# YongonY/NBLDPC

Measured on AMD Instinct MI355X. Metric: decoded codewords/sec @ 50 iters, GF(256) N=512 rate-1/2, higher is better.
Workload: dtype f64

## Files before the change

### nbldpc_amd/csrc/nbl_cn_ems256.hip

```cpp
#include <hip/hip_runtime.h>
#ifndef NBL_EMS_PRUNE
#define NBL_EMS_PRUNE 1
#endif
#ifndef NBL_EMS_ND
#define NBL_EMS_ND 1
#endif
#include <type_traits>
#include "nbl_device.h"
#include "nbl_kernels.h"

#ifndef NBL_WHATIF
#define NBL_WHATIF 0
#endif

namespace {

constexpr int Q = 256;

struct ListEnt { double v; int t8; int tt; };

#define WSYNC() __builtin_amdgcn_fence(__ATOMIC_ACQ_REL, "wavefront")

template <int CTRL, int ROW_MASK = 0xF>
__device__ __forceinline__ double dpp_mov_f64(double x)
{
	int lo = __builtin_amdgcn_update_dpp(__double2loint(x), __double2loint(x), CTRL, ROW_MASK, 0xF, false);
	int hi = __builtin_amdgcn_update_dpp(__double2hiint(x), __double2hiint(x), CTRL, ROW_MASK, 0xF, false);
	return __hiloint2double(hi, lo);
}

__device__ __forceinline__ double wave_max_f64(double x)
{
	x = dmax(x, dpp_mov_f64<0xB1>(x));
	x = dmax(x, dpp_mov_f64<0x4E>(x));
	x = dmax(x, dpp_mov_f64<0x141>(x));
	x = dmax(x, dpp_mov_f64<0x140>(x));
	x = dmax(x, dpp_mov_f64<0x142, 0xA>(x));
	x = dmax(x, dpp_mov_f64<0x143, 0xC>(x));
	return read_lane_f64(x, 63);
}

__device__ __forceinline__ int wave_scan_add(int x)
{
	x += __builtin_amdgcn_update_dpp(0, x, 0x111, 0xF, 0xF, false);
	x += __builtin_amdgcn_update_dpp(0, x, 0x112, 0xF, 0xF, false);
	x += __builtin_amdgcn_update_dpp(0, x, 0x114, 0xF, 0xF, false);
	x += __builtin_amdgcn_update_dpp(0, x, 0x118, 0xF, 0xF, false);
	x += __builtin_amdgcn_update_dpp(0, x, 0x142, 0xA, 0xF, false);
	x += __builtin_amdgcn_update_dpp(0, x, 0x143, 0xC, 0xF, false);
	return x;
}

__device__ __forceinline__ int wave_max_i32(int x)
{
	constexpr int ID = (int)0x80000000;
	auto mx = [](int a, int b) { return a > b ? a : b; };
	x = mx(x, __builtin_amdgcn_update_dpp(ID, x, 0xB1, 0xF, 0xF, false));
	x = mx(x, __builtin_amdgcn_update_dpp(ID, x, 0x4E, 0xF, 0xF, false));
	x = mx(x, __builtin_amdgcn_update_dpp(ID, x, 0x141, 0xF, 0xF, false));
	x = mx(x, __builtin_amdgcn_update_dpp(ID, x, 0x140, 0xF, 0xF, false));
	x = mx(x, __builtin_amdgcn_update_dpp(ID, x, 0x142, 0xA, 0xF, false));
	x = mx(x, __builtin_amdgcn_update_dpp(ID, x, 0x143, 0xC, 0xF, false));
	return __builtin_amdgcn_readlane(x, 63);
}
__device__ __forceinline__ int wave_min_i32(int x)
{
	constexpr int ID = 0x7fffffff;
	auto mn = [](int a, int b) { return a < b ? a : b; };
	x = mn(x, __builtin_amdgcn_update_dpp(ID, x, 0xB1, 0xF, 0xF, false));
	x = mn(x, __builtin_amdgcn_update_dpp(ID, x, 0x4E, 0xF, 0xF, false));
	x = mn(x, __builtin_amdgcn_update_dpp(ID, x, 0x141, 0xF, 0xF, false));
	x = mn(x, __builtin_amdgcn_update_dpp(ID, x, 0x140, 0xF, 0xF, false));
	x = mn(x, __builtin_amdgcn_update_dpp(ID, x, 0x142, 0xA, 0xF, false));
	x = mn(x, __builtin_amdgcn_update_dpp(ID, x, 0x143, 0xC, 0xF, false));
	return __builtin_amdgcn_readlane(x, 63);
}

__device__ __forceinline__ int key32(double x)
{
	const int b = __float_as_int((float)x);
	return b ^ ((b >> 31) & 0x7fffffff);
}
__device__ __forceinline__ float unkey32(int k) { return __int_as_float(k ^ ((k >> 31) & 0x7fffffff)); }

__device__ __forceinline__ double wave_max_exact(double loc, int key, int kmax)
{
	const uint64_t c = __ballot(key == kmax);
	if (__builtin_popcountll(c) == 1) return read_lane_f64(loc, __builtin_ctzll(c));
	return wave_max_f64(loc);
}

__device__ __forceinline__ int sym_of(int lane, int i) { return 2 * lane + (i & 1) + 128 * (i >> 1); }

__device__ __forceinline__ int highest_sym(const uint64_t (&m)[4])
{
	int best = -1;
#pragma unroll
	for (int i = 0; i < 4; i++) {
		if (m[i]) {
			int l = 63 - __builtin_clzll(m[i]);
			int a = 2 * l + (i & 1) + 128 * (i >> 1);
			best = a > best ? a : best;
		}
	}
	return best;
}
__device__ __forceinline__ int lowest_sym(const uint64_t (&m)[4])
{
	int best = Q;
#pragma unroll
	for (int i = 0; i < 4; i++) {
		if (m[i]) {
			int l = __builtin_ctzll(m[i]);
			int a = 2 * l + (i & 1) + 128 * (i >> 1);
			best = a < best ? a : best;
		}
	}
	return best;
}

struct GfMulL {
	int b0, b7, lane_part;
	__device__ __forceinline__ void init(int h, int poly, int lane)
	{
		int x = h;
		b0 = x;
		lane_part = 0;
#pragma unroll
		for (int i = 1; i < 8; i++) {
			x <<= 1;
			if (x & Q) x ^= poly;
			if (i < 7) lane_part ^= (-((lane >> (i - 1)) & 1)) & x;
			else b7 = x;
		}
	}
	__device__ __forceinline__ int at_slot(int i) const { return lane_part ^ ((i & 1) ? b0 : 0) ^ ((i & 2) ? b7 : 0); }
};

struct SelState {
	uint64_t cand[4];
	uint64_t gt[4], eq[4];
	int done;
};

__device__ __forceinline__ void select_step(const double (&v)[4], int nm, SelState &s)
{
	if (s.done) return;
	const uint64_t any = s.cand[0] | s.cand[1] | s.cand[2] | s.cand[3];
	if (!any) { s.done = 1; return; }
	double offer = __builtin_amdgcn_inverse_ballot_w64(s.cand[0]) ? v[0] : __builtin_amdgcn_inverse_ballot_w64(s.cand[1]) ? v[1]
	             : __builtin_amdgcn_inverse_ballot_w64(s.cand[2]) ? v[2] : v[3];
	const double pv = read_lane_f64(offer, __builtin_ctzll(any));
	uint64_t gt[4], ge[4];
	int cgt = 0, cge = 0;
#pragma unroll
	for (int i = 0; i < 4; i++) {
		gt[i] = __ballot(v[i] > pv);
		ge[i] = __ballot(v[i] >= pv);
		cgt += __popcll(gt[i]);
		cge += __popcll(ge[i]);
	}
	if (cgt >= nm) {
#pragma unroll
		for (int i = 0; i < 4; i++) s.cand[i] &= gt[i];
	} else if (cge >= nm) {
#pragma unroll
		for (int i = 0; i < 4; i++) { s.gt[i] = gt[i]; s.eq[i] = ge[i] & ~gt[i]; }
		s.done = 1;
	} else {
#pragma unroll
		for (int i = 0; i < 4; i++) s.cand[i] &= ~ge[i];
	}
}

__device__ __forceinline__ void finish_ties(uint64_t (&member)[4], const uint64_t (&eqin)[4], int need, int hinv, int poly, int lane)
{
	GfMulL mh;
	mh.init(hinv, poly, lane);
	uint64_t eq[4] = {eqin[0], eqin[1], eqin[2], eqin[3]};
	for (; need > 0; need--) {
		int best = -1;
#pragma unroll
		for (int i = 0; i < 4; i++) {
			const int a = __builtin_amdgcn_inverse_ballot_w64(eq[i]) ? mh.at_slot(i) : -1;
			best = a > best ? a : best;
		}
		const int amax = wave_max_i32(best);
#pragma unroll
		for (int i = 0; i < 4; i++) {
			const uint64_t hit = __ballot(__builtin_amdgcn_inverse_ballot_w64(eq[i]) && mh.at_slot(i) == amax);
			member[i] |= hit;
			eq[i] &= ~hit;
		}
	}
}

__device__ __forceinline__ void finish_members(SelState &s, int nm, uint64_t (&member)[4], int hinv, int poly, int lane)
{
	int cgt = 0, ceq = 0;
#pragma unroll
	for (int i = 0; i < 4; i++) { cgt += __popcll(s.gt[i]); ceq += __popcll(s.eq[i]); }
	const int need = nm - cgt;
#pragma unroll
	for (int i = 0; i < 4; i++) member[i] = s.gt[i];
	if (need == ceq) {
#pragma unroll
		for (int i = 0; i < 4; i++) member[i] |= s.eq[i];
	} else {
		finish_ties(member, s.eq, need, hinv, poly, lane);
	}
}

}

template <int NMT, bool FUSED, int NC>
__global__ __launch_bounds__(64) void cn_ems_q256_dc4_kernel(NblGraphDev g, NblWork w, NblRun r)
{
	constexpr int NM = NMT < 0 ? -NMT : NMT;
	constexpr bool VARNM = NMT < 0;
	const int nmr = VARNM ? r.nm : NM;
	constexpr int LOGNM = (NM == 8) ? 3 : (NM == 16) ? 4 : (NM == 32) ? 5 : 6;
#if NBL_WHATIF == 5
	__shared__ __attribute__((aligned(16))) char smem[13 * 1024];
#elif NBL_WHATIF == 6
	__shared__ __attribute__((aligned(16))) char smem[19 * 1024];
#else
	__shared__ __attribute__((aligned(16))) char smem[3 * Q * 8 + 4 * NM * 8 + 4 * NM * 8];
#endif
	const int lane = lane_id();
	const NblXcdSlot xs = nbl_xcd_slot(g.M);
	const int m = xs.unit, b = nbl_codeword(w, r, xs.slot);
	if (b < 0) return;
	if (!r.fixed_iters && w.done[b]) return;
#if NBL_EMS_PRUNE
	const bool tryf = NC >= 2 && r.fixed_iters && w.done[b];
#else
	const bool tryf = false;
#endif
	const int c0 = g.coff[m];

	double *const B0 = (double *)smem, *const B1 = B0 + Q, *const B2 = B1 + Q;
	double *const lstv = B2 + Q;
	int2 *const lstt = (int2 *)(lstv + 4 * NM);
	auto list_at = [&](int j, int k) {
		ListEnt e;
		e.v = lstv[j * NM + k];
		const int2 o = lstt[j * NM + k];
		e.t8 = o.x;
		e.tt = o.y;
		return e;
	};

#ifdef NBL_EMS_STAMPS
	unsigned long long st_t0 = 0, st_acc[15] = {0, 0, 0, 0, 0, 0, 0, 0, 0, 0, 0, 0, 0, 0, 0};
	const bool st_on = (w.stamps != nullptr) && ((blockIdx.x & 63) == 0);
#define STAMP(i) do { if (st_on) { unsigned long long t1_ = clock64(); st_acc[i] += t1_ - st_t0; st_t0 = t1_; } } while (0)
#define STAMP_COUNT(i) do { if (st_on) st_acc[i]++; } while (0)
	const unsigned long long st_begin = st_on ? clock64() : 0;
	unsigned long long st_mid = 0;
	int st_cls = 6;
	st_t0 = st_begin;
#elif defined(NBL_EMS_MARKS)
#define STAMP(i) asm volatile("; NBLMARK " #i)
#define STAMP_COUNT(i) do { } while (0)
#else
#define STAMP(i) do { } while (0)
#define STAMP_COUNT(i) do { } while (0)
#endif

	const double *V = w.v2c + (size_t)b * g.E * Q;
	double *C = w.c2v + ((size_t)b * g.E + c0) * Q;

	uint2 toff[4];
#define TOFF(j, i) ((int)((((i) & 2) ? toff[j].y : toff[j].x) >> (16 * ((i) & 1))) & 0xffff)
#pragma unroll
	for (int j = 0; j < 4; j++) toff[j] = ((const uint2 *)g.ems_toff)[(size_t)(c0 + j) * 64 + lane];

	double v[4][4];
	if (!FUSED) {
#pragma unroll
		for (int j = 0; j < 4; j++) {
			const double2 *src = (const double2 *)(V + (size_t)g.c_epos[c0 + j] * Q);
			double2 d0 = src[lane], d1 = src[64 + lane];
			v[j][0] = (lane == 0) ? 0.0 : d0.x;
			v[j][1] = d0.y;
			v[j][2] = d1.x;
			v[j][3] = d1.y;
		}
	} else {
		const double *Cp = w.c2v_prev + (w.c2v_prev_shared ? (size_t)0 : (size_t)b * g.E * Q);
		double2 l0[4], l1[4], a0[4], a1[4], b0[4], b1[4];
		int nvar[4], eidx[4];
		bool ownA[4];
		const int *row = g.dv2_row + (size_t)m * 16;
#pragma unroll
		for (int j = 0; j < 4; j++) {
			const int n = row[j], cpA = row[4 + j], cpB = row[8 + j], e = row[12 + j] & 0x7fffffff;
#if NBL_WHATIF == 11
			const double2 *pl = (const double2 *)(w.Lch + ((size_t)(b & 7) * g.N + n) * Q);
#else
			const double2 *pl = (const double2 *)(w.Lch + ((size_t)b * g.N + n) * Q);
#endif
			const double2 *pa = (const double2 *)(Cp + (size_t)cpA * Q);
			const double2 *pb = (const double2 *)(Cp + (size_t)cpB * Q);
#if NBL_WHATIF == 4
			l0[j].x = (double)(long long)(pl + lane) * -1e-9; l0[j].y = l0[j].x * 1.5; l1[j].x = l0[j].x * 0.7; l1[j].y = l0[j].x * 0.3;
			a0[j].x = (double)(long long)(pa + lane) * -1e-9; a0[j].y = a0[j].x * 1.25; a1[j].x = a0[j].x * 0.6; a1[j].y = a0[j].x * 0.2;
			b0[j].x = (double)(long long)(pb + lane) * -1e-9; b0[j].y = b0[j].x * 1.125; b1[j].x = b0[j].x * 0.9; b1[j].y = b0[j].x * 0.4;
#else
			l0[j] = pl[lane]; l1[j] = pl[64 + lane];
			a0[j] = pa[lane]; a1[j] = pa[64 + lane];
			b0[j] = pb[lane]; b1[j] = pb[64 + lane];
#endif
			nvar[j] = n; eidx[j] = e;
			ownA[j] = row[12 + j] < 0;
		}
#pragma unroll
		for (int j = 0; j < 4; j++) {
			const int n = nvar[j], e = eidx[j];
			double post[4] = {(l0[j].x + a0[j].x) + b0[j].x, (l0[j].y + a0[j].y) + b0[j].y, (l1[j].x + a1[j].x) + b1[j].x,
			                  (l1[j].y + a1[j].y) + b1[j].y};
			if (ownA[j]) {
				v[j][0] = post[0] - a0[j].x; v[j][1] = post[1] - a0[j].y; v[j][2] = post[2] - a1[j].x; v[j][3] = post[3] - a1[j].y;
			} else {
				asm volatile("");
				v[j][0] = post[0] - b0[j].x; v[j][1] = post[1] - b0[j].y; v[j][2] = post[2] - b1[j].x; v[j][3] = post[3] - b1[j].y;
			}
			if (lane == 0) v[j][0] = 0.0;
			if (ownA[j]) {
				if (lane == 0) post[0] = 0.0;
				const double locp = dmax(dmax(post[0], post[1]), dmax(post[2], post[3]));
				const int kp = key32(locp);
				const double pm = wave_max_exact(locp, kp, wave_max_i32(kp));
				uint64_t hit[4];
#pragma unroll
				for (int i = 0; i < 4; i++) hit[i] = __ballot(post[i] == pm);
				const int arg = lowest_sym(hit);
				if (lane == 0) w.dec[(size_t)b * g.N + n] = (pm > 0.0) ? arg : 0;
				if (w.post) {
					double2 *pp = (double2 *)(w.post + ((size_t)b * g.N + n) * Q);
					double2 p01, p23;
					p01.x = post[0]; p01.y = post[1]; p23.x = post[2]; p23.y = post[3];
					pp[lane] = p01;
					pp[64 + lane] = p23;
				}
			}
			if (w.store_v2c) {
				double2 *pv = (double2 *)(w.v2c + ((size_t)b * g.E + e) * Q);
				double2 v01, v23;
				v01.x = v[j][0]; v01.y = v[j][1]; v23.x = v[j][2]; v23.y = v[j][3];
				pv[lane] = v01;
				pv[64 + lane] = v23;
			}
		}
	}
	STAMP(0);

	double mtop[4], lmin[4];
	double sec[4] = {0, 0, 0, 0};
	int ztop[4];
#pragma unroll
	for (int j = 0; j < 4; j++) {
		const double loc = dmax(dmax(v[j][0], v[j][1]), dmax(v[j][2], v[j][3]));
		const int k = key32(loc);
		mtop[j] = wave_max_exact(loc, k, wave_max_i32(k));
		constexpr int KEY_3E38 = 0x7f61b1e6;
		const int kmin = wave_min_i32(k);
		const double lf = (double)unkey32(kmin < KEY_3E38 ? kmin : KEY_3E38);
		lmin[j] = ((lf - (mtop[j] - lf) * 0x1p-20) - __builtin_fabs(lf) * 0x1p-22) - 0x1p-120;
		uint64_t eqm[4];
#pragma unroll
		for (int i = 0; i < 4; i++) eqm[i] = __ballot(v[j][i] == mtop[j]);
		const int topa = highest_sym(eqm);
		const int tl = (topa & 127) >> 1;
		const unsigned twl = (unsigned)__builtin_amdgcn_readlane((int)toff[j].x, tl), twh = (unsigned)__builtin_amdgcn_readlane((int)toff[j].y, tl);
		const unsigned tw = (topa & 128) ? twh : twl;
		ztop[j] = (int)((tw >> (16 * (topa & 1))) & 0xffffu) >> 3;
#if NBL_EMS_PRUNE
		if (tryf) {
			const int ts = (topa & 1) + 2 * (topa >> 7);
			const double mate = (ts == 0) ? v[j][1] : (ts == 1) ? v[j][0] : (ts == 2) ? v[j][3] : v[j][2];
			const double far = (ts & 2) ? dmax(v[j][0], v[j][1]) : dmax(v[j][2], v[j][3]);
			const double loc2 = (lane == tl) ? dmax(mate, far) : loc;
			const double sf = (double)unkey32(wave_max_i32(key32(loc2)));
			sec[j] = uniform_f64((sf + __builtin_fabs(sf) * 0x1p-22) + 0x1p-120);
		}
#endif
	}
	STAMP(1);

	double S[4][4];
#pragma unroll
	for (int x = 0; x < 4; x++)
#pragma unroll
		for (int i = 0; i < 4; i++) S[x][i] = -NBL_DBL_MAX;
	const int ztot = ztop[0] ^ ztop[1] ^ ztop[2] ^ ztop[3];
	const int lane16 = lane << 4;
#pragma unroll
	for (int j = 0; j < 4; j++) {
		char *const Uj = (char *)(j == 1 ? B1 : j == 2 ? B2 : B0);
		WSYNC();
#pragma unroll
		for (int i = 0; i < 4; i++) *(double *)(Uj + TOFF(j, i)) = v[j][i];
		WSYNC();
#pragma unroll
		for (int x = 0; x < 4; x++) {
			if (x == j) continue;
			const int shift = ztot ^ ztop[x] ^ ztop[j];
			const int ad = lane16 ^ ((shift & 0xFE) << 3);
			const double2 ra = *(const double2 *)(Uj + ad), rb = *(const double2 *)(Uj + (ad ^ 1024));
			auto upd = [&](double u0, double u1, double u2, double u3) {
				const double uu[4] = {u0, u1, u2, u3};
#pragma unroll
				for (int i = 0; i < 4; i++) {
					double acc = 0.0;
#pragma unroll
					for (int o = 0; o < 4; o++) {
						if (o == x) continue;
						acc = acc + ((o == j) ? uu[i] : mtop[o]);
					}
					S[x][i] = dmax(S[x][i], acc);
				}
			};
			if (shift & 1) upd(ra.y, ra.x, rb.y, rb.x);
			else upd(ra.x, ra.y, rb.x, rb.y);
		}
		if (NC >= 2) {
			const double2 d0 = *(const double2 *)(Uj + lane16), d1 = *(const double2 *)(Uj + lane16 + 1024);
			v[j][0] = d0.x; v[j][1] = d0.y; v[j][2] = d1.x; v[j][3] = d1.y;
		}
	}
	STAMP(5);

	int n0[4] = {0, 0, 0, 0}, nA[4] = {0, 0, 0, 0}, nC[4] = {0, 0, 0, 0};
	int cntl[4] = {nmr, nmr, nmr, nmr};
	bool fast = false;
	int nd = 4;
	double thr[4] = {0, 0, 0, 0};
#if NBL_EMS_PRUNE
	if (tryf) {
		double flo[4];
#pragma unroll
		for (int x = 0; x < 4; x++) {
			const double lf = (double)unkey32(wave_min_i32(key32(dmin(dmin(S[x][0], S[x][1]), dmin(S[x][2], S[x][3])))));
			flo[x] = uniform_f64((lf - __builtin_fabs(lf) * 0x1p-22) - 0x1p-120);
		}
		auto pb = [&](int b, int c) { return dmax(mtop[b] + sec[c], sec[b] + mtop[c]); };
		const double p01 = pb(0, 1), p02 = pb(0, 2), p03 = pb(0, 3), p12 = pb(1, 2), p13 = pb(1, 3), p23 = pb(2, 3);
		auto low = [&](double f, double p) {
			const double t = f - p;
			return (t - (__builtin_fabs(f) + __builtin_fabs(p)) * 0x1p-40) - 0x1p-100;
		};
		thr[0] = uniform_f64(dmin(dmin(low(flo[1], p23), low(flo[2], p13)), low(flo[3], p12)));
		thr[1] = uniform_f64(dmin(dmin(low(flo[0], p23), low(flo[2], p03)), low(flo[3], p02)));
		thr[2] = uniform_f64(dmin(dmin(low(flo[0], p13), low(flo[1], p03)), low(flo[3], p01)));
		thr[3] = uniform_f64(dmin(dmin(low(flo[0], p12), low(flo[1], p02)), low(flo[2], p01)));
		fast = true;
#pragma unroll
		for (int j = 0; j < 4; j++) {
			int c = 0;
#pragma unroll
			for (int i = 0; i < 4; i++) c += __popcll(__ballot(!(v[j][i] < thr[j])));
			cntl[j] = c;
			fast = fast && c <= nmr;
		}
		nd = (cntl[0] >= 2) + (cntl[1] >= 2) + (cntl[2] >= 2) + (cntl[3] >= 2);
		if (!fast) { cntl[0] = cntl[1] = cntl[2] = cntl[3] = nmr; nd = 4; }
#ifdef NBL_EMS_STAMPS
		if (st_on) { st_acc[13] += fast ? 1 : 0; st_acc[14] += cntl[0] + cntl[1] + cntl[2] + cntl[3]; }
		if (w.stamps) st_cls = fast ? nd : 5;
#endif
	}
#endif
#ifdef NBL_EMS_STAMPS
	if (st_on) st_mid = clock64();
#endif
	constexpr int ND_SKIP = NBL_EMS_ND ? 1 : -1;
	const bool skip_held = !FUSED && NBL_EMS_ND && fast && nd <= 1;
#define ND_SKIPPED (FUSED ? nd <= ND_SKIP : skip_held)
#define ND_KEPT (FUSED ? nd > ND_SKIP : !skip_held)
	if (NC >= 2 && ND_KEPT) {
		auto compact = [&](int j, const uint64_t (&member)[4]) {
			const int c0n = __popcll(member[0]), c2n = __popcll(member[2]), c1n = __popcll(member[1]);
			const int ne = c0n + c2n;
			n0[j] = ne;
			nA[j] = c0n;
			nC[j] = ne + c1n;
			const int base[4] = {j * NM, j * NM + ne, j * NM + c0n, j * NM + ne + c1n};
#pragma unroll
			for (int i = 0; i < 4; i++) {
				const int pos = __builtin_amdgcn_mbcnt_hi((uint32_t)(member[i] >> 32), __builtin_amdgcn_mbcnt_lo((uint32_t)member[i], base[i]));
				if (__builtin_amdgcn_inverse_ballot_w64(member[i])) {
					lstv[pos] = v[j][i];
					lstt[pos] = make_int2(sym_of(lane, i) << 3, (sym_of(lane, i) & 0x7E) << 3);
				}
			}
		};
		if (VARNM || fast) {
			WSYNC();
#pragma unroll
			for (int j = 0; j < 4; j++) {
				lstv[j * NM + (lane & (NM - 1))] = NBL_NEG_INF;
				lstt[j * NM + (lane & (NM - 1))] = make_int2((lane & (NM - 1)) << 3, 0);
			}
			WSYNC();
		}
		if (fast) {
#pragma unroll
			for (int j = 0; j < 4; j++) {
				uint64_t member[4];
#pragma unroll
				for (int i = 0; i < 4; i++) member[i] = __ballot(!(v[j][i] < thr[j]));
				compact(j, member);
			}
		} else {
			int bk[4][4];
			int *H = (int *)B0;
			int one;
			asm volatile("v_mov_b32 %0, 1" : "=v"(one));
			WSYNC();
			{
				int4 z4 = {0, 0, 0, 0};
#pragma unroll
				for (int i = 0; i < 4; i++) ((int4 *)H)[i * 64 + lane] = z4;
			}
			WSYNC();
#pragma unroll
			for (int j = 0; j < 4; j++) {
				const double scale = 256.0 * __builtin_amdgcn_rcp(mtop[j] - lmin[j]);
#pragma unroll
				for (int i = 0; i < 4; i++) {
					int bi;
					asm("v_cvt_i32_f64 %0, %1" : "=v"(bi) : "v"((mtop[j] - v[j][i]) * scale));
					bk[j][i] = bi;
					if (bi < 256) __hip_atomic_fetch_add(&H[j * 256 + bi], one, __ATOMIC_RELAXED, __HIP_MEMORY_SCOPE_WORKGROUP);
				}
			}
			WSYNC();
			int hc[4][4];
#pragma unroll
			for (int j = 0; j < 4; j++) {
				const int4 h4 = ((int4 *)H)[j * 64 + lane];
				hc[0][j] = h4.x; hc[1][j] = h4.y; hc[2][j] = h4.z; hc[3][j] = h4.w;
			}
			STAMP(2);
#pragma unroll
			for (int j = 0; j < 4; j++) {
				uint64_t member[4];
				const int tot = hc[0][j] + hc[1][j] + hc[2][j] + hc[3][j];
				const int cum = wave_scan_add(tot);
				const uint64_t reach = __ballot(cum >= nmr);
				const int lstar = reach ? __builtin_ctzll(reach) : 63;
				const int cl = __builtin_amdgcn_readlane(cum, lstar);
				const int q1 = __builtin_amdgcn_readlane(hc[1][j], lstar),
				          q2 = __builtin_amdgcn_readlane(hc[2][j], lstar), q3 = __builtin_amdgcn_readlane(hc[3][j], lstar);
				const int s0 = cl - q3 - q2 - q1, s1 = cl - q3 - q2, s2 = cl - q3;
				const int bsel = (s0 >= nmr) ? 0 : (s1 >= nmr) ? 1 : (s2 >= nmr) ? 2 : 3;
				const int upto = (s0 >= nmr) ? s0 : (s1 >= nmr) ? s1 : (s2 >= nmr) ? s2 : cl;
				const int bstar = 4 * lstar + bsel;
				const bool exact = reach && upto == nmr;
				if (exact) {
#pragma unroll
					for (int i = 0; i < 4; i++) member[i] = __ballot(bk[j][i] <= bstar);
				} else {
					STAMP_COUNT(10);
					SelState ss;
#pragma unroll
					for (int i = 0; i < 4; i++) { ss.cand[i] = reach ? __ballot(bk[j][i] == bstar) : ~0ull; ss.gt[i] = ss.eq[i] = 0; }
					ss.done = 0;
					for (int guard = 0; guard < 300 && !ss.done; guard++) {
						select_step(v[j], nmr, ss);
						STAMP_COUNT(9);
					}
					finish_members(ss, nmr, member, g.c_hinv[c0 + j], g.poly, lane);
				}
				compact(j, member);
			}
		}
	}
	WSYNC();
	STAMP(4);

	constexpr int PER = 64 >> LOGNM, ROUNDS = (NM << LOGNM) >> 6;
	const int rounds = VARNM ? (nmr + PER - 1) >> (6 - LOGNM) : ROUNDS;
	const int apos = (lane & 1) ? (NM - 1) - ((lane & (NM - 1)) >> 1) : ((lane & (NM - 1)) >> 1);
	auto pair_scatter = [&](double *dst, int ja, int jb, double bias, int sxor) __attribute__((always_inline)) {
		WSYNC();
		double2 ninf;
		ninf.x = NBL_NEG_INF;
		ninf.y = NBL_NEG_INF;
		((double2 *)dst)[lane] = ninf;
		((double2 *)dst)[64 + lane] = ninf;
		ListEnt ea = list_at(ja, apos);
		ea.v = ea.v + bias;
		ea.t8 ^= sxor << 3;
		WSYNC();
		if (fast) {
			for (int it = 0, nit = __builtin_amdgcn_readfirstlane((cntl[jb] + PER - 1) >> (6 - LOGNM)); it < nit; it++) {
				const ListEnt eb = list_at(jb, it * PER + (lane >> LOGNM));
				__hip_atomic_fetch_max((double *)((char *)dst + (ea.t8 ^ eb.t8)), ea.v + eb.v, __ATOMIC_RELAXED, __HIP_MEMORY_SCOPE_WORKGROUP);
			}
		} else
#pragma unroll
		for (int it = 0; it < rounds; it++) {
			const ListEnt eb = list_at(jb, it * PER + (lane >> LOGNM));
			__hip_atomic_fetch_max((double *)((char *)dst + (ea.t8 ^ eb.t8)), ea.v + eb.v, __ATOMIC_RELAXED, __HIP_MEMORY_SCOPE_WORKGROUP);
		}
		WSYNC();
	};
	auto pair_scatter_more = [&](double *dst, int ja, int jb, double bias, int sxor) __attribute__((always_inline)) {
		ListEnt ea = list_at(ja, apos);
		ea.v = ea.v + bias;
		ea.t8 ^= sxor << 3;
		if (fast) {
			for (int it = 0, nit = __builtin_amdgcn_readfirstlane((cntl[jb] + PER - 1) >> (6 - LOGNM)); it < nit; it++) {
				const ListEnt eb = list_at(jb, it * PER + (lane >> LOGNM));
				__hip_atomic_fetch_max((double *)((char *)dst + (ea.t8 ^ eb.t8)), ea.v + eb.v, __ATOMIC_RELAXED, __HIP_MEMORY_SCOPE_WORKGROUP);
			}
		} else
#pragma unroll
		for (int it = 0; it < rounds; it++) {
			const ListEnt eb = list_at(jb, it * PER + (lane >> LOGNM));
			__hip_atomic_fetch_max((double *)((char *)dst + (ea.t8 ^ eb.t8)), ea.v + eb.v, __ATOMIC_RELAXED, __HIP_MEMORY_SCOPE_WORKGROUP);
		}
		WSYNC();
	};
	auto fold = [&](const double *src, int sx, double add, double (&Sout)[4]) {
		const char *Sb = (const char *)src;
		const int ad = lane16 ^ ((sx & 0xFE) << 3);
		const double2 ra = *(const double2 *)(Sb + ad), rb = *(const double2 *)(Sb + (ad ^ 1024));
		const bool sw = sx & 1;
		Sout[0] = dmax(Sout[0], (sw ? ra.y : ra.x) + add);
		Sout[1] = dmax(Sout[1], (sw ? ra.x : ra.y) + add);
		Sout[2] = dmax(Sout[2], (sw ? rb.y : rb.x) + add);
		Sout[3] = dmax(Sout[3], (sw ? rb.x : rb.y) + add);
	};
	auto conf_nc2 = [&](int x, int o1, int o2, int o3) {
		fold(B0, ztop[o3], mtop[o3], S[x]);
		pair_scatter(B1, o2, o3, mtop[o1], ztop[o1]);
		pair_scatter_more(B1, o1, o3, mtop[o2], ztop[o2]);
		{
			const double2 ra = ((const double2 *)B1)[lane], rb = ((const double2 *)B1)[64 + lane];
			S[x][0] = dmax(S[x][0], ra.x); S[x][1] = dmax(S[x][1], ra.y);
			S[x][2] = dmax(S[x][2], rb.x); S[x][3] = dmax(S[x][3], rb.y);
		}
	};
	auto gather_conv = [&](int jc, auto np_tag, double (&acc)[decltype(np_tag)::value][4]) {
		constexpr int NP = decltype(np_tag)::value;
		constexpr int UN = 4;
		const char *Pb = (const char *)B0;
		auto body = [&](const ListEnt &en, auto swapped, auto upper) {
			constexpr bool SW = decltype(swapped)::value, HI = decltype(upper)::value;
#if NBL_WHATIF == 10
			const int ad = en.tt & 1008;
#else
			const int ad = lane16 ^ en.tt;
#endif
			double2 ra[NP], rb[NP];
#pragma unroll
			for (int p = 0; p < NP; p++) {
#if NBL_WHATIF == 1
				ra[p].x = acc[p][1]; ra[p].y = acc[p][0]; rb[p].x = acc[p][3]; rb[p].y = acc[p][2];
				asm volatile("" : "+v"(ra[p].x), "+v"(ra[p].y), "+v"(rb[p].x), "+v"(rb[p].y) : "v"(ad));
#else
				ra[p] = *(const double2 *)(Pb + p * (Q * 8) + ad + (HI ? 1024 : 0));
				rb[p] = *(const double2 *)(Pb + p * (Q * 8) + ad + (HI ? 0 : 1024));
#endif
			}
#pragma unroll
			for (int p = 0; p < NP; p++) {
#if NBL_WHATIF == 2
				acc[p][0] = dmax(acc[p][0], (SW ? ra[p].y : ra[p].x));
				acc[p][1] = dmax(acc[p][1], (SW ? ra[p].x : ra[p].y));
				acc[p][2] = dmax(acc[p][2], (SW ? rb[p].y : rb[p].x));
				acc[p][3] = dmax(acc[p][3], (SW ? rb[p].x : rb[p].y));
#else
				acc[p][0] = dmax(acc[p][0], (SW ? ra[p].y : ra[p].x) + en.v);
				acc[p][1] = dmax(acc[p][1], (SW ? ra[p].x : ra[p].y) + en.v);
				acc[p][2] = dmax(acc[p][2], (SW ? rb[p].y : rb[p].x) + en.v);
				acc[p][3] = dmax(acc[p][3], (SW ? rb[p].x : rb[p].y) + en.v);
#endif
			}
		};
		const double myv = lstv[jc * NM + (lane & (NM - 1))];
		const int mytt = lstt[jc * NM + (lane & (NM - 1))].y;
		auto entry = [&](int k) {
			ListEnt e;
			e.v = read_lane_f64(myv, k);
			e.tt = __builtin_amdgcn_readlane(mytt, k);
			e.t8 = 0;
			return e;
		};
		auto run = [&](int k0, int k1, auto swapped, auto upper) {
			int k = k0;
			for (; k + UN <= k1; k += UN) {
				STAMP_COUNT(11);
				ListEnt en[UN];
#pragma unroll
				for (int u = 0; u < UN; u++) en[u] = entry(k + u);
#pragma unroll
				for (int u = 0; u < UN; u++) body(en[u], swapped, upper);
			}
			for (; k < k1; k++) { STAMP_COUNT(12); body(entry(k), swapped, upper); }
		};
		const int eA = __builtin_amdgcn_readfirstlane(nA[jc]), e0 = __builtin_amdgcn_readfirstlane(n0[jc]), eC = __builtin_amdgcn_readfirstlane(nC[jc]), eN = __builtin_amdgcn_readfirstlane(cntl[jc]);
		run(0, eA, std::false_type{}, std::false_type{});
		run(eA, e0, std::false_type{}, std::true_type{});
		run(e0, eC, std::true_type{}, std::false_type{});
		run(eC, eN, std::true_type{}, std::true_type{});
	};
	auto emit_stage = [&](int x, double *Sx) {
		double2 s01, s23;
		s01.x = S[x][0]; s01.y = S[x][1]; s23.x = S[x][2]; s23.y = S[x][3];
		((double2 *)Sx)[lane] = s01;
		((double2 *)Sx)[64 + lane] = s23;
	};
	auto emit_store = [&](int x, const double *Sx) {
		const double s0 = Sx[0];
		double y[4];
#pragma unroll
		for (int i = 0; i < 4; i++) y[i] = shape_llr(*(const double *)((const char *)Sx + TOFF(x, i)) - s0, r.factor, r.offset);
		if (lane == 0) y[0] = 0.0;
		double2 o01, o23;
		o01.x = y[0]; o01.y = y[1]; o23.x = y[2]; o23.y = y[3];
		double2 *dst = (double2 *)(C + (size_t)x * Q);
		dst[lane] = o01;
		dst[64 + lane] = o23;
	};

	if (ND_SKIPPED) {
	} else if (NC >= 3) {
		{
			double2 ninf;
			ninf.x = NBL_NEG_INF;
			ninf.y = NBL_NEG_INF;
#pragma unroll
			for (int i = 0; i < 6; i++) ((double2 *)B0)[i * 64 + lane] = ninf;
			const ListEnt ea0 = list_at(0, apos), ea1 = list_at(1, apos);
			WSYNC();
			if (fast) {
				const int mc = cntl[1] > cntl[2] ? cntl[1] : cntl[2];
				for (int it = 0, nit = __builtin_amdgcn_readfirstlane((mc + PER - 1) >> (6 - LOGNM)); it < nit; it++) {
					const ListEnt eb1 = list_at(1, it * PER + (lane >> LOGNM)), eb2 = list_at(2, it * PER + (lane >> LOGNM));
					__hip_atomic_fetch_max((double *)((char *)B0 + (ea0.t8 ^ eb1.t8)), ea0.v + eb1.v, __ATOMIC_RELAXED, __HIP_MEMORY_SCOPE_WORKGROUP);
					__hip_atomic_fetch_max((double *)((char *)B1 + (ea0.t8 ^ eb2.t8)), ea0.v + eb2.v, __ATOMIC_RELAXED, __HIP_MEMORY_SCOPE_WORKGROUP);
					__hip_atomic_fetch_max((double *)((char *)B2 + (ea1.t8 ^ eb2.t8)), ea1.v + eb2.v, __ATOMIC_RELAXED, __HIP_MEMORY_SCOPE_WORKGROUP);
				}
			} else
#pragma unroll
			for (int it = 0; it < rounds; it++) {
				const ListEnt eb1 = list_at(1, it * PER + (lane >> LOGNM)), eb2 = list_at(2, it * PER + (lane >> LOGNM));
#if NBL_WHATIF == 3
				double keep = (ea0.v + eb1.v) + ((ea0.v + eb2.v) + (ea1.v + eb2.v));
				int keepa = (ea0.t8 ^ eb1.t8) + (ea0.t8 ^ eb2.t8) + (ea1.t8 ^ eb2.t8);
				asm volatile("" : : "v"(keep), "v"(keepa));
#elif NBL_WHATIF == 7
				*(volatile double *)((char *)B0 + (ea0.t8 ^ eb1.t8)) = ea0.v + eb1.v;
				*(volatile double *)((char *)B1 + (ea0.t8 ^ eb2.t8)) = ea0.v + eb2.v;
				*(volatile double *)((char *)B2 + (ea1.t8 ^ eb2.t8)) = ea1.v + eb2.v;
#else
				__hip_atomic_fetch_max((double *)((char *)B0 + (ea0.t8 ^ eb1.t8)), ea0.v + eb1.v, __ATOMIC_RELAXED, __HIP_MEMORY_SCOPE_WORKGROUP);
				__hip_atomic_fetch_max((double *)((char *)B1 + (ea0.t8 ^ eb2.t8)), ea0.v + eb2.v, __ATOMIC_RELAXED, __HIP_MEMORY_SCOPE_WORKGROUP);
				__hip_atomic_fetch_max((double *)((char *)B2 + (ea1.t8 ^ eb2.t8)), ea1.v + eb2.v, __ATOMIC_RELAXED, __HIP_MEMORY_SCOPE_WORKGROUP);
#endif
			}
			WSYNC();
		}
		STAMP(6);
		{
			double a3[1][4], a210[3][4];
#pragma unroll
			for (int i = 0; i < 4; i++) { a3[0][i] = S[3][i]; a210[0][i] = S[2][i]; a210[1][i] = S[1][i]; a210[2][i] = S[0][i]; }
			gather_conv(2, std::integral_constant<int, 1>{}, a3);
			gather_conv(3, std::integral_constant<int, 3>{}, a210);
#pragma unroll
			for (int i = 0; i < 4; i++) { S[3][i] = a3[0][i]; S[2][i] = a210[0][i]; S[1][i] = a210[1][i]; S[0][i] = a210[2][i]; }
		}
		STAMP(7);
	} else if (NC == 2) {
		pair_scatter(B0, 0, 1, 0.0, 0);
		conf_nc2(3, 0, 1, 2);
		conf_nc2(2, 0, 1, 3);
		pair_scatter(B0, 0, 2, 0.0, 0);
		conf_nc2(1, 0, 2, 3);
		pair_scatter(B0, 1, 2, 0.0, 0);
		conf_nc2(0, 1, 2, 3);
		STAMP(6);
	}
	WSYNC();
#ifdef NBL_EMS_STAMPS
	const unsigned long long st_emit = st_on ? clock64() : 0;
#endif
	emit_stage(3, B0);
	emit_stage(2, B1);
	emit_stage(1, B2);
	WSYNC();
	emit_store(3, B0);
	emit_store(2, B1);
	emit_store(1, B2);
	WSYNC();
	emit_stage(0, B0);
	WSYNC();
	emit_store(0, B0);
	STAMP(8);

#ifdef NBL_EMS_STAMPS
	if (st_on && lane == 0) {
		for (int i = 0; i < 15; i++) atomicAdd(&w.stamps[i], st_acc[i]);
		atomicAdd(&w.stamps[15], 1ull);
		atomicAdd(&w.stamps[16 + st_cls], 1ull);
		atomicAdd(&w.stamps[24 + st_cls], st_t0 - st_begin);
		atomicAdd(&w.stamps[32 + st_cls], st_emit - st_mid);
	}
	if (w.stamps && lane == 0) atomicAdd(&w.stamps[40 + st_cls], 1ull);
#endif
#undef STAMP
#undef STAMP_COUNT
#undef TOFF
#undef ND_SKIPPED
#undef ND_KEPT
}

bool nbl_ems256_applicable(const NblShape &s, int nm, int nc)
{
	return s.has_ems_toff() && nc >= 1 && nm >= 1 && nm <= 64;
}

size_t nbl_ems256_lds_bytes(int nm) { return 3 * Q * 8 + (size_t)4 * (nm <= 8 ? 8 : nm <= 16 ? 16 : nm <= 32 ? 32 : 64) * 16; }

template <int NM, bool FUSED>
static void launch_nc(int nc, dim3 grid, dim3 block, hipStream_t st, const NblGraphDev &g, const NblWork &w, const NblRun &r)
{
	if (nc >= 3) cn_ems_q256_dc4_kernel<NM, FUSED, 3><<<grid, block, 0, st>>>(g, w, r);
	else if (nc == 2) cn_ems_q256_dc4_kernel<NM, FUSED, 2><<<grid, block, 0, st>>>(g, w, r);
	else cn_ems_q256_dc4_kernel<NM, FUSED, 1><<<grid, block, 0, st>>>(g, w, r);
}

hipError_t nbl_launch_cn_ems256(const NblGraphDev &g, const NblWork &w, const NblRun &r, bool fused, hipStream_t st)
{
	dim3 grid(nbl_xcd_grid(r.B, g.M)), block(64);
	if (fused) {
		switch (r.nm) {
		case 8: launch_nc<8, true>(r.nc, grid, block, st, g, w, r); break;
		case 16: launch_nc<16, true>(r.nc, grid, block, st, g, w, r); break;
		case 32: launch_nc<32, true>(r.nc, grid, block, st, g, w, r); break;
		case 64: launch_nc<64, true>(r.nc, grid, block, st, g, w, r); break;
		default:
			if (r.nm < 8) launch_nc<-8, true>(r.nc, grid, block, st, g, w, r);
			else if (r.nm < 16) launch_nc<-16, true>(r.nc, grid, block, st, g, w, r);
			else if (r.nm < 32) launch_nc<-32, true>(r.nc, grid, block, st, g, w, r);
			else launch_nc<-64, true>(r.nc, grid, block, st, g, w, r);
			break;
		}
	} else {
		switch (r.nm) {
		case 8: launch_nc<8, false>(r.nc, grid, block, st, g, w, r); break;
		case 16: launch_nc<16, false>(r.nc, grid, block, st, g, w, r); break;
		case 32: launch_nc<32, false>(r.nc, grid, block, st, g, w, r); break;
		case 64: launch_nc<64, false>(r.nc, grid, block, st, g, w, r); break;
		default:
			if (r.nm < 8) launch_nc<-8, false>(r.nc, grid, block, st, g, w, r);
			else if (r.nm < 16) launch_nc<-16, false>(r.nc, grid, block, st, g, w, r);
			else if (r.nm < 32) launch_nc<-32, false>(r.nc, grid, block, st, g, w, r);
			else launch_nc<-64, false>(r.nc, grid, block, st, g, w, r);
			break;
		}
	}
	return hipGetLastError();
}
```

### nbldpc_amd/csrc/nbl_device.h

```cpp
#pragma once
#include <hip/hip_runtime.h>
#include "nbl_common.h"

#define NBL_NEG_INF (-__builtin_huge_val())
#define NBL_DBL_MAX 1.7976931348623157e308

template <int Q> struct Fld {
	static constexpr int NS = (Q + 63) / 64;
	static constexpr int P = (Q == 4) ? 2 : (Q == 8) ? 3 : (Q == 16) ? 4 : (Q == 32) ? 5 : (Q == 64) ? 6 : (Q == 128) ? 7 : 8;
};

__device__ __forceinline__ int lane_id() { return threadIdx.x & 63; }

struct NblXcdSlot { int slot, unit; };
__device__ __forceinline__ NblXcdSlot nbl_xcd_slot(int units)
{
	const int xcd = blockIdx.x & 7, idx = blockIdx.x >> 3;
	NblXcdSlot s;
	s.slot = (idx / units) * 8 + xcd;
	s.unit = idx % units;
	return s;
}
inline unsigned nbl_xcd_grid(int B, int units) { return (unsigned)((long long)((B + 7) / 8) * 8 * units); }

__device__ __forceinline__ int nbl_codeword(const NblWork &w, const NblRun &r, int slot)
{
	if (slot >= r.B) return -1;
	if (!w.active) return slot;
	return slot < *w.n_act ? w.active[slot] : -1;
}

__device__ __forceinline__ double dmax(double a, double b)
{
	double r;
	asm("v_max_f64 %0, %1, %2" : "=v"(r) : "v"(a), "v"(b));
	return r;
}
__device__ __forceinline__ double dmin(double a, double b)
{
	double r;
	asm("v_min_f64 %0, %1, %2" : "=v"(r) : "v"(a), "v"(b));
	return r;
}

__device__ __forceinline__ double read_lane_f64(double v, int lane)
{
	int lo = __builtin_amdgcn_readlane(__double2loint(v), lane);
	int hi = __builtin_amdgcn_readlane(__double2hiint(v), lane);
	return __hiloint2double(hi, lo);
}

template <int CTRL, int ROW_MASK> __device__ __forceinline__ int dpp_i32(int v)
{
	return __builtin_amdgcn_update_dpp(v, v, CTRL, ROW_MASK, 0xF, false);
}
template <int CTRL, int ROW_MASK> __device__ __forceinline__ double dpp_f64(double v)
{
	return __hiloint2double(dpp_i32<CTRL, ROW_MASK>(__double2hiint(v)), dpp_i32<CTRL, ROW_MASK>(__double2loint(v)));
}
__device__ __forceinline__ double wave_fmax(double v)
{
	v = dmax(v, dpp_f64<0x111, 0xF>(v));
	v = dmax(v, dpp_f64<0x112, 0xF>(v));
	v = dmax(v, dpp_f64<0x114, 0xF>(v));
	v = dmax(v, dpp_f64<0x118, 0xF>(v));
	v = dmax(v, dpp_f64<0x142, 0xA>(v));
	v = dmax(v, dpp_f64<0x143, 0xC>(v));
	return read_lane_f64(v, 63);
}
__device__ __forceinline__ double wave_fmin(double v)
{
	v = dmin(v, dpp_f64<0x111, 0xF>(v));
	v = dmin(v, dpp_f64<0x112, 0xF>(v));
	v = dmin(v, dpp_f64<0x114, 0xF>(v));
	v = dmin(v, dpp_f64<0x118, 0xF>(v));
	v = dmin(v, dpp_f64<0x142, 0xA>(v));
	v = dmin(v, dpp_f64<0x143, 0xC>(v));
	return read_lane_f64(v, 63);
}
__device__ __forceinline__ int wave_imax(int v)
{
	v = max(v, dpp_i32<0x111, 0xF>(v));
	v = max(v, dpp_i32<0x112, 0xF>(v));
	v = max(v, dpp_i32<0x114, 0xF>(v));
	v = max(v, dpp_i32<0x118, 0xF>(v));
	v = max(v, dpp_i32<0x142, 0xA>(v));
	v = max(v, dpp_i32<0x143, 0xC>(v));
	return __builtin_amdgcn_readlane(v, 63);
}

__device__ __forceinline__ int nbl_key32(double x)
{
	const int b = __float_as_int((float)x);
	return b ^ ((b >> 31) & 0x7fffffff);
}
__device__ __forceinline__ float nbl_unkey32(int k) { return __int_as_float(k ^ ((k >> 31) & 0x7fffffff)); }
__device__ __forceinline__ int wave_imax_id(int x)
{
	constexpr int ID = (int)0x80000000;
	x = max(x, __builtin_amdgcn_update_dpp(ID, x, 0x111, 0xF, 0xF, false));
	x = max(x, __builtin_amdgcn_update_dpp(ID, x, 0x112, 0xF, 0xF, false));
	x = max(x, __builtin_amdgcn_update_dpp(ID, x, 0x114, 0xF, 0xF, false));
	x = max(x, __builtin_amdgcn_update_dpp(ID, x, 0x118, 0xF, 0xF, false));
	x = max(x, __builtin_amdgcn_update_dpp(ID, x, 0x142, 0xA, 0xF, false));
	x = max(x, __builtin_amdgcn_update_dpp(ID, x, 0x143, 0xC, 0xF, false));
	return __builtin_amdgcn_readlane(x, 63);
}

__device__ __forceinline__ unsigned wave_umax_id(unsigned x)
{
	x = max(x, (unsigned)__builtin_amdgcn_update_dpp(0, (int)x, 0x111, 0xF, 0xF, false));
	x = max(x, (unsigned)__builtin_amdgcn_update_dpp(0, (int)x, 0x112, 0xF, 0xF, false));
	x = max(x, (unsigned)__builtin_amdgcn_update_dpp(0, (int)x, 0x114, 0xF, 0xF, false));
	x = max(x, (unsigned)__builtin_amdgcn_update_dpp(0, (int)x, 0x118, 0xF, 0xF, false));
	x = max(x, (unsigned)__builtin_amdgcn_update_dpp(0, (int)x, 0x142, 0xA, 0xF, false));
	x = max(x, (unsigned)__builtin_amdgcn_update_dpp(0, (int)x, 0x143, 0xC, 0xF, false));
	return (unsigned)__builtin_amdgcn_readlane((int)x, 63);
}
__device__ __forceinline__ double wave_fmax_nonneg(double x)
{
	x = dmax(x, 0.0);
	const unsigned hi = (unsigned)__double2hiint(x), mh = wave_umax_id(hi);
	const unsigned lo = (hi == mh) ? (unsigned)__double2loint(x) : 0u, ml = wave_umax_id(lo);
	return __hiloint2double((int)mh, (int)ml);
}

__device__ __forceinline__ unsigned wave_umin_id(unsigned x)
{
	constexpr int ID = -1;
	x = min(x, (unsigned)__builtin_amdgcn_update_dpp(ID, (int)x, 0x111, 0xF, 0xF, false));
	x = min(x, (unsigned)__builtin_amdgcn_update_dpp(ID, (int)x, 0x112, 0xF, 0xF, false));
	x = min(x, (unsigned)__builtin_amdgcn_update_dpp(ID, (int)x, 0x114, 0xF, 0xF, false));
	x = min(x, (unsigned)__builtin_amdgcn_update_dpp(ID, (int)x, 0x118, 0xF, 0xF, false));
	x = min(x, (unsigned)__builtin_amdgcn_update_dpp(ID, (int)x, 0x142, 0xA, 0xF, false));
	x = min(x, (unsigned)__builtin_amdgcn_update_dpp(ID, (int)x, 0x143, 0xC, 0xF, false));
	return (unsigned)__builtin_amdgcn_readlane((int)x, 63);
}
__device__ __forceinline__ double wave_fmin_nonneg(double x)
{
	const unsigned hi = (unsigned)__double2hiint(x), mh = wave_umin_id(hi);
	const unsigned lo = (hi == mh) ? (unsigned)__double2loint(x) : 0xffffffffu, ml = wave_umin_id(lo);
	return __hiloint2double((int)mh, (int)ml);
}

__device__ __forceinline__ int uniform(int v) { return __builtin_amdgcn_readfirstlane(v); }

__device__ __forceinline__ double uniform_f64(double v)
{
	return __hiloint2double(__builtin_amdgcn_readfirstlane(__double2hiint(v)),
	                        __builtin_amdgcn_readfirstlane(__double2loint(v)));
}

__device__ __forceinline__ int prefix_count(uint64_t mask)
{
	return __builtin_amdgcn_mbcnt_hi((uint32_t)(mask >> 32), __builtin_amdgcn_mbcnt_lo((uint32_t)mask, 0));
}

template <int Q> struct GfMul {
	int basis[8];
	int lane_part;
	__device__ __forceinline__ void init(int h, int poly, int lane)
	{
		int x = h;
#pragma unroll
		for (int i = 0; i < 8; i++) {
			basis[i] = x;
			x <<= 1;
			if (x & Q) x ^= poly;
		}
		lane_part = 0;
#pragma unroll
		for (int i = 0; i < 6; i++)
			if (i < Fld<Q>::P) lane_part ^= (-((lane >> i) & 1)) & basis[i];
	}
	__device__ __forceinline__ int at_slot(int slot) const
	{
		int t = lane_part;
		if (slot & 1) t ^= basis[6];
		if (slot & 2) t ^= basis[7];
		return t;
	}
};

template <int NS> __device__ __forceinline__ int wave_decide(const double (&v)[NS], int lane, int q)
{
	double best = 0.0;
#pragma unroll
	for (int i = 0; i < NS; i++)
		if (lane + 64 * i < q) best = dmax(best, v[i]);
	if (!__ballot(best > 0.0)) return 0;
	const double mx = wave_fmax_nonneg(best);
	int arg = 0;
#pragma unroll
	for (int i = NS - 1; i >= 0; i--) {
		const uint64_t hit = __ballot(lane + 64 * i < q && v[i] == mx);
		arg = hit ? 64 * i + __builtin_ctzll(hit) : arg;
	}
	return arg;
}

template <int NS> __device__ __forceinline__ int wave_decide_keyed(const double (&v)[NS], int lane, int q)
{
	double best = 0.0;
#pragma unroll
	for (int i = 0; i < NS; i++)
		if (lane + 64 * i < q) best = dmax(best, v[i]);
	if (!__ballot(best > 0.0)) return 0;
	const int k = nbl_key32(best), kmax = wave_imax_id(k);
	const uint64_t c = __ballot(k == kmax);
	const double mx = (__builtin_popcountll(c) == 1) ? read_lane_f64(best, __builtin_ctzll(c)) : wave_fmax(best);
	int arg = 0;
#pragma unroll
	for (int i = NS - 1; i >= 0; i--) {
		const uint64_t hit = __ballot(lane + 64 * i < q && v[i] == mx);
		arg = hit ? 64 * i + __builtin_ctzll(hit) : arg;
	}
	return arg;
}

__device__ __forceinline__ double shape_llr(double y, double factor, double offset)
{
	if (factor == 1.0 && offset == 0.0) return (y < 0.0 || y > 0.0) ? y : 0.0;
	if (factor != 1.0) y = y / factor;
	if (y < -1 * offset) return y + offset;
	if (y > offset) return y - offset;
	return 0.0;
}
```

Before: 122,100.

## Batch wave reductions four-wide, defer lmin, add early fast path and packed offsets

Replaces per-row serial DPP max/min reductions with a four-way interleaved reduction so the independent DPP chains overlap instead of serialising on latency. Moves the lmin computation into the slow branch that actually uses it, adds a shortcut that marks all rows as single-candidate when every second-best lies below its threshold (skipping the ballot counts), and packs four list-entry offsets into one lane word so each unrolled group needs one readlane instead of four. Trades some register pressure and extra DPP shifts for fewer serial reduction stalls and fewer scalar reads.

```diff
diff --git a/nbldpc_amd/csrc/nbl_cn_ems256.hip b/nbldpc_amd/csrc/nbl_cn_ems256.hip
--- a/nbldpc_amd/csrc/nbl_cn_ems256.hip
+++ b/nbldpc_amd/csrc/nbl_cn_ems256.hip
@@ -4,6 +4,9 @@
 #endif
 #ifndef NBL_EMS_ND
 #define NBL_EMS_ND 1
+#endif
+#ifndef NBL_EMS_TRIMS
+#define NBL_EMS_TRIMS 13
 #endif
 #include <type_traits>
 #include "nbl_device.h"
@@ -61,18 +64,6 @@
 	x = mx(x, __builtin_amdgcn_update_dpp(ID, x, 0x140, 0xF, 0xF, false));
 	x = mx(x, __builtin_amdgcn_update_dpp(ID, x, 0x142, 0xA, 0xF, false));
 	x = mx(x, __builtin_amdgcn_update_dpp(ID, x, 0x143, 0xC, 0xF, false));
-	return __builtin_amdgcn_readlane(x, 63);
-}
-__device__ __forceinline__ int wave_min_i32(int x)
-{
-	constexpr int ID = 0x7fffffff;
-	auto mn = [](int a, int b) { return a < b ? a : b; };
-	x = mn(x, __builtin_amdgcn_update_dpp(ID, x, 0xB1, 0xF, 0xF, false));
-	x = mn(x, __builtin_amdgcn_update_dpp(ID, x, 0x4E, 0xF, 0xF, false));
-	x = mn(x, __builtin_amdgcn_update_dpp(ID, x, 0x141, 0xF, 0xF, false));
-	x = mn(x, __builtin_amdgcn_update_dpp(ID, x, 0x140, 0xF, 0xF, false));
-	x = mn(x, __builtin_amdgcn_update_dpp(ID, x, 0x142, 0xA, 0xF, false));
-	x = mn(x, __builtin_amdgcn_update_dpp(ID, x, 0x143, 0xC, 0xF, false));
 	return __builtin_amdgcn_readlane(x, 63);
 }
 
@@ -359,31 +350,57 @@
 	double mtop[4], lmin[4];
 	double sec[4] = {0, 0, 0, 0};
 	int ztop[4];
-#pragma unroll
-	for (int j = 0; j < 4; j++) {
-		const double loc = dmax(dmax(v[j][0], v[j][1]), dmax(v[j][2], v[j][3]));
-		const int k = key32(loc);
-		mtop[j] = wave_max_exact(loc, k, wave_max_i32(k));
+	auto lmin_of = [](int kmin, double mt) {
 		constexpr int KEY_3E38 = 0x7f61b1e6;
-		const int kmin = wave_min_i32(k);
 		const double lf = (double)unkey32(kmin < KEY_3E38 ? kmin : KEY_3E38);
-		lmin[j] = ((lf - (mtop[j] - lf) * 0x1p-20) - __builtin_fabs(lf) * 0x1p-22) - 0x1p-120;
-		uint64_t eqm[4];
-#pragma unroll
-		for (int i = 0; i < 4; i++) eqm[i] = __ballot(v[j][i] == mtop[j]);
-		const int topa = highest_sym(eqm);
-		const int tl = (topa & 127) >> 1;
-		const unsigned twl = (unsigned)__builtin_amdgcn_readlane((int)toff[j].x, tl), twh = (unsigned)__builtin_amdgcn_readlane((int)toff[j].y, tl);
-		const unsigned tw = (topa & 128) ? twh : twl;
-		ztop[j] = (int)((tw >> (16 * (topa & 1))) & 0xffffu) >> 3;
+		return ((lf - (mt - lf) * 0x1p-20) - __builtin_fabs(lf) * 0x1p-22) - 0x1p-120;
+	};
+	{
+		double loc[4];
+		int kj[4], kmax[4], tlj[4], topaj[4];
+#pragma unroll
+		for (int j = 0; j < 4; j++) {
+			loc[j] = dmax(dmax(v[j][0], v[j][1]), dmax(v[j][2], v[j][3]));
+			kmax[j] = kj[j] = key32(loc[j]);
+		}
+		wave_reduce_i32x4<true>(kmax);
+#if !(NBL_EMS_TRIMS & 4)
+		int kmin[4] = {kj[0], kj[1], kj[2], kj[3]};
+		wave_reduce_i32x4<false>(kmin);
+#endif
+#pragma unroll
+		for (int j = 0; j < 4; j++) {
+			mtop[j] = wave_max_exact(loc[j], kj[j], kmax[j]);
+#if !(NBL_EMS_TRIMS & 4)
+			lmin[j] = lmin_of(kmin[j], mtop[j]);
+#endif
+			uint64_t eqm[4];
+#pragma unroll
+			for (int i = 0; i < 4; i++) eqm[i] = __ballot(v[j][i] == mtop[j]);
+			const int topa = highest_sym(eqm);
+			const int tl = (topa & 127) >> 1;
+			const unsigned twl = (unsigned)__builtin_amdgcn_readlane((int)toff[j].x, tl), twh = (unsigned)__builtin_amdgcn_readlane((int)toff[j].y, tl);
+			const unsigned tw = (topa & 128) ? twh : twl;
+			ztop[j] = (int)((tw >> (16 * (topa & 1))) & 0xffffu) >> 3;
+			topaj[j] = topa;
+			tlj[j] = tl;
+		}
 #if NBL_EMS_PRUNE
 		if (tryf) {
-			const int ts = (topa & 1) + 2 * (topa >> 7);
-			const double mate = (ts == 0) ? v[j][1] : (ts == 1) ? v[j][0] : (ts == 2) ? v[j][3] : v[j][2];
-			const double far = (ts & 2) ? dmax(v[j][0], v[j][1]) : dmax(v[j][2], v[j][3]);
-			const double loc2 = (lane == tl) ? dmax(mate, far) : loc;
-			const double sf = (double)unkey32(wave_max_i32(key32(loc2)));
-			sec[j] = uniform_f64((sf + __builtin_fabs(sf) * 0x1p-22) + 0x1p-120);
+			int k2[4];
+#pragma unroll
+			for (int j = 0; j < 4; j++) {
+				const int ts = (topaj[j] & 1) + 2 * (topaj[j] >> 7);
+				const double mate = (ts == 0) ? v[j][1] : (ts == 1) ? v[j][0] : (ts == 2) ? v[j][3] : v[j][2];
+				const double far = (ts & 2) ? dmax(v[j][0], v[j][1]) : dmax(v[j][2], v[j][3]);
+				k2[j] = key32((lane == tlj[j]) ? dmax(mate, far) : loc[j]);
+			}
+			wave_reduce_i32x4<true>(k2);
+#pragma unroll
+			for (int j = 0; j < 4; j++) {
+				const double sf = (double)unkey32(k2[j]);
+				sec[j] = uniform_f64((sf + __builtin_fabs(sf) * 0x1p-22) + 0x1p-120);
+			}
 		}
 #endif
 	}
@@ -440,9 +457,13 @@
 #if NBL_EMS_PRUNE
 	if (tryf) {
 		double flo[4];
+		int kf[4];
+#pragma unroll
+		for (int x = 0; x < 4; x++) kf[x] = key32(dmin(dmin(S[x][0], S[x][1]), dmin(S[x][2], S[x][3])));
+		wave_reduce_i32x4<false>(kf);
 #pragma unroll
 		for (int x = 0; x < 4; x++) {
-			const double lf = (double)unkey32(wave_min_i32(key32(dmin(dmin(S[x][0], S[x][1]), dmin(S[x][2], S[x][3])))));
+			const double lf = (double)unkey32(kf[x]);
 			flo[x] = uniform_f64((lf - __builtin_fabs(lf) * 0x1p-22) - 0x1p-120);
 		}
 		auto pb = [&](int b, int c) { return dmax(mtop[b] + sec[c], sec[b] + mtop[c]); };
@@ -456,16 +477,24 @@
 		thr[2] = uniform_f64(dmin(dmin(low(flo[0], p13), low(flo[1], p03)), low(flo[3], p01)));
 		thr[3] = uniform_f64(dmin(dmin(low(flo[0], p12), low(flo[1], p02)), low(flo[2], p01)));
 		fast = true;
-#pragma unroll
-		for (int j = 0; j < 4; j++) {
-			int c = 0;
-#pragma unroll
-			for (int i = 0; i < 4; i++) c += __popcll(__ballot(!(v[j][i] < thr[j])));
-			cntl[j] = c;
-			fast = fast && c <= nmr;
-		}
-		nd = (cntl[0] >= 2) + (cntl[1] >= 2) + (cntl[2] >= 2) + (cntl[3] >= 2);
-		if (!fast) { cntl[0] = cntl[1] = cntl[2] = cntl[3] = nmr; nd = 4; }
+#if (NBL_EMS_TRIMS & 8) && NBL_EMS_ND
+		if ((sec[0] < thr[0]) & (sec[1] < thr[1]) & (sec[2] < thr[2]) & (sec[3] < thr[3])) {
+			cntl[0] = cntl[1] = cntl[2] = cntl[3] = 1;
+			nd = 0;
+		} else
+#endif
+		{
+#pragma unroll
+			for (int j = 0; j < 4; j++) {
+				int c = 0;
+#pragma unroll
+				for (int i = 0; i < 4; i++) c += __popcll(__ballot(!(v[j][i] < thr[j])));
+				cntl[j] = c;
+				fast = fast && c <= nmr;
+			}
+			nd = (cntl[0] >= 2) + (cntl[1] >= 2) + (cntl[2] >= 2) + (cntl[3] >= 2);
+			if (!fast) { cntl[0] = cntl[1] = cntl[2] = cntl[3] = nmr; nd = 4; }
+		}
 #ifdef NBL_EMS_STAMPS
 		if (st_on) { st_acc[13] += fast ? 1 : 0; st_acc[14] += cntl[0] + cntl[1] + cntl[2] + cntl[3]; }
 		if (w.stamps) st_cls = fast ? nd : 5;
@@ -518,6 +547,16 @@
 			int *H = (int *)B0;
 			int one;
 			asm volatile("v_mov_b32 %0, 1" : "=v"(one));
+#if NBL_EMS_TRIMS & 4
+			{
+				int kmin[4];
+#pragma unroll
+				for (int j = 0; j < 4; j++) kmin[j] = key32(dmax(dmax(v[j][0], v[j][1]), dmax(v[j][2], v[j][3])));
+				wave_reduce_i32x4<false>(kmin);
+#pragma unroll
+				for (int j = 0; j < 4; j++) lmin[j] = lmin_of(kmin[j], mtop[j]);
+			}
+#endif
 			WSYNC();
 			{
 				int4 z4 = {0, 0, 0, 0};
@@ -683,11 +722,21 @@
 			}
 		};
 		const double myv = lstv[jc * NM + (lane & (NM - 1))];
-		const int mytt = lstt[jc * NM + (lane & (NM - 1))].y;
+		int mytt = lstt[jc * NM + (lane & (NM - 1))].y;
+#if NBL_EMS_TRIMS & 1
+		{
+			auto next_lane = [](int x) { return __builtin_amdgcn_update_dpp(0, x, 0x130, 0xF, 0xF, true); };
+			const int t1 = next_lane(mytt), t2 = next_lane(t1), t3 = next_lane(t2);
+			mytt |= (t1 << 6) | (t2 << 12) | (t3 << 18);
+		}
+#endif
 		auto entry = [&](int k) {
 			ListEnt e;
 			e.v = read_lane_f64(myv, k);
 			e.tt = __builtin_amdgcn_readlane(mytt, k);
+#if NBL_EMS_TRIMS & 1
+			e.tt &= 0x3F0;
+#endif
 			e.t8 = 0;
 			return e;
 		};
@@ -696,8 +745,19 @@
 			for (; k + UN <= k1; k += UN) {
 				STAMP_COUNT(11);
 				ListEnt en[UN];
+#if NBL_EMS_TRIMS & 1
+				static_assert(UN == 4, "one packed word holds the offsets of four entries");
+				const int w4 = __builtin_amdgcn_readlane(mytt, k);
+#pragma unroll
+				for (int u = 0; u < UN; u++) {
+					en[u].v = read_lane_f64(myv, k + u);
+					en[u].tt = (w4 >> (6 * u)) & 0x3F0;
+					en[u].t8 = 0;
+				}
+#else
 #pragma unroll
 				for (int u = 0; u < UN; u++) en[u] = entry(k + u);
+#endif
 #pragma unroll
 				for (int u = 0; u < UN; u++) body(en[u], swapped, upper);
 			}
diff --git a/nbldpc_amd/csrc/nbl_device.h b/nbldpc_amd/csrc/nbl_device.h
--- a/nbldpc_amd/csrc/nbl_device.h
+++ b/nbldpc_amd/csrc/nbl_device.h
@@ -107,6 +107,24 @@
 	return __builtin_amdgcn_readlane(x, 63);
 }
 
+template <bool MAX> __device__ __forceinline__ void wave_reduce_i32x4(int (&x)[4])
+{
+	constexpr int ID = MAX ? (int)0x80000000 : 0x7fffffff;
+	auto op = [](int a, int b) { return MAX ? (a > b ? a : b) : (a < b ? a : b); };
+	__builtin_amdgcn_sched_barrier(0);
+#define NBL_RED4_STEP(CTRL, ROWS)                                                                                      \
+	_Pragma("unroll") for (int i = 0; i < 4; i++) x[i] = op(x[i], __builtin_amdgcn_update_dpp(ID, x[i], CTRL, ROWS, 0xF, false));
+	NBL_RED4_STEP(0xB1, 0xF)
+	NBL_RED4_STEP(0x4E, 0xF)
+	NBL_RED4_STEP(0x141, 0xF)
+	NBL_RED4_STEP(0x140, 0xF)
+	NBL_RED4_STEP(0x142, 0xA)
+	NBL_RED4_STEP(0x143, 0xC)
+#undef NBL_RED4_STEP
+#pragma unroll
+	for (int i = 0; i < 4; i++) x[i] = __builtin_amdgcn_readlane(x[i], 63);
+}
+
 __device__ __forceinline__ unsigned wave_umax_id(unsigned x)
 {
 	x = max(x, (unsigned)__builtin_amdgcn_update_dpp(0, (int)x, 0x111, 0xF, 0xF, false));
```

Result: faster. 123,400, median of 6 (+1.0%).
